# Acelogic/LTX-2-MLX

Measured on AMD Instinct MI355X. Metric: denoise_steps_per_sec, higher is better.
Workload: dtype bf16; 1 GPU; LTX-2 19B distilled DiT (48 layers, D=4096, 32x128 heads), 768x512x65 (N=3456 video tokens, S=1024 text tokens), 8-step distilled sigmas, bf16, random-init weights; parallelism=prompt-parallel x1 (independent prompt/seed per GPU, one RCCL weight broadcast)

## Files before the change

### ltx-2-mlx_amd/csrc/gemm_v4.hip

```cpp
#include <stdlib.h>

#include "gemm_epilogue.h"
#include "gemm_v4_loop.inc"

namespace {

typedef unsigned int u32x8 __attribute__((ext_vector_type(8)));
typedef unsigned int u32x16 __attribute__((ext_vector_type(16)));

#define V4_INS_DENSE : "{v[0:15]}"(voffA), "{v[16:23]}"(voffB), "{v[24:27]}"(addrA), "{v[28:31]}"(addrB), [ra] "s"(ra), [rw] "s"(rw), \
                       [nk] "s"(nk), [la] "s"(la), [lw] "s"(lw), [kb] "s"(kb)
#define V4_INS_CONV V4_INS_DENSE, "{v32}"(tapv), [lcpt] "s"(lcpt), [cptm1] "s"(cptm1)
#define V4_OUT16                                                                                                          \
    "={a[0:15]}"(acc[0]), "={a[16:31]}"(acc[1]), "={a[32:47]}"(acc[2]), "={a[48:63]}"(acc[3]), "={a[64:79]}"(acc[4]),   \
        "={a[80:95]}"(acc[5]), "={a[96:111]}"(acc[6]), "={a[112:127]}"(acc[7]), "={a[128:143]}"(acc[8]),                 \
        "={a[144:159]}"(acc[9]), "={a[160:175]}"(acc[10]), "={a[176:191]}"(acc[11]), "={a[192:207]}"(acc[12]),          \
        "={a[208:223]}"(acc[13]), "={a[224:239]}"(acc[14]), "={a[240:255]}"(acc[15])
#define V4_ASM(LOOP) asm volatile(LOOP : V4_OUT16 V4_INS_DENSE : LTX2_V4_CLOBBERS)
#define V4_ASM_CONV(LOOP) asm volatile(LOOP : V4_OUT16 V4_INS_CONV : LTX2_V4_CLOBBERS)

template <int LAYOUT, int BM, bool W8 = false>
struct V4Geo {
    static constexpr bool L41 = LAYOUT == 4 || LAYOUT == 7;
    static constexpr int BN = LAYOUT == 4 ? 128 : LAYOUT == 7 ? 64 : 256;
    static_assert(LAYOUT == 3 || LAYOUT == 4 || LAYOUT == 5 || LAYOUT == 6 || LAYOUT == 7, "wave layout");
    static constexpr int MB = LAYOUT == 5 ? 32 : 16;
    static constexpr bool L14 = !L41;
    static constexpr int WM = L41 ? BM / 4 : BM;
    static constexpr int WN = LAYOUT == 4 ? 128 : 64;
    static constexpr int RBW = (WM + MB - 1) / MB, CBW = WN / MB;
    static constexpr int NKS = MB == 16 ? 2 : 4;
    static constexpr int WROW = W8 ? 64 : 128;
    static constexpr int NPA = BM / 32, NPW = BN * WROW / 4096;
    static constexpr int A_STAGE = L41 ? BM * 128 : 32768, W_BASE = 2 * A_STAGE, W_STAGE = BN * WROW;
    static_assert(!W8 || LAYOUT == 3, "fp8-resident weights run on layout 3");
    static constexpr int LOOP_BYTES = W_BASE + 2 * W_STAGE;
    static constexpr int EPI_BYTES = 4 * WM * WN * 2;
    static constexpr int LDS_BYTES = LOOP_BYTES > EPI_BYTES ? LOOP_BYTES : EPI_BYTES;
    static_assert(LAYOUT == 4 ? (BM == 384 || BM == 448 || BM == 512) : LAYOUT == 7 ? BM == 512 : (BM == 224 || BM == 256), "tile rows");
    static_assert(LAYOUT != 6 || BM == 224, "layout 6 tile rows");
    static_assert(LDS_BYTES <= 160 * 1024, "LDS");
};

template <int EPI, int LAYOUT, int BM, bool CONV, int VAR>
__device__ __forceinline__ void gemm_v4_tile(const GemmParams& p, const int bid) {
    constexpr bool W8 = VAR == 20;
    constexpr bool F8 = LAYOUT == 5 || LAYOUT == 6;
    using G = V4Geo<LAYOUT, BM, W8>;
    constexpr int TBN = G::BN, NPA = G::NPA, NPW = G::NPW, MB = G::MB, WM = G::WM, WN = G::WN, RBW = G::RBW, CBW = G::CBW, NKS = G::NKS;
    static_assert(!CONV || !(LAYOUT == 5 || LAYOUT == 6), "conv runs on the bf16 layouts");
    extern __shared__ __attribute__((aligned(16))) char smem[];
    const unsigned lds0 = (unsigned)(uintptr_t)(lds_ptr_t)smem;
    const int tid = threadIdx.x;
    const int lane = tid & 63;
    const int w = __builtin_amdgcn_readfirstlane(tid >> 6);
    const int wr = G::L41 ? w : 0, wc = G::L41 ? 0 : w;
#ifdef LTX2_V4_PROBE
    const unsigned long long t_k0 = __builtin_amdgcn_s_memtime();
#endif

    constexpr bool FOLD_OK = LAYOUT == 3 && !CONV && VAR == 30;
    constexpr bool FOLD_CONS = FOLD_OK && (EPI == EPI_BF16 || EPI == EPI_GELU_BF16);
    constexpr bool FOLD_PROD = FOLD_OK && EPI == EPI_RESID_GATE_F32;
    const int Mt = (p.M + BM - 1) / BM, Nt = LAYOUT == 7 ? 1 : p.N / TBN;
    const int ntiles = Mt * Nt;
    const int split = p.splitk > 1 ? bid / ntiles : 0;
    const int id = xcd_remap(bid - split * ntiles, ntiles);
    constexpr int GROUP = 8;
    const int per_group = GROUP * Nt;
    const int g = id / per_group;
    const int first_m = g * GROUP;
    const int gsz = min(Mt - first_m, GROUP);
    const int rem = id - g * per_group;
    const int m0 = (first_m + rem % gsz) * BM;
    const int n0 = (rem / gsz) * TBN;

    u32x16 voffA = {0, 0, 0, 0, 0, 0, 0, 0, 0, 0, 0, 0, 0, 0, 0, 0};
    u32x8 voffB = {0, 0, 0, 0, 0, 0, 0, 0};
    const int Hp = p.H + 2, Wp = p.Wd + 2;
    constexpr bool SHORT_OK = LAYOUT == 3 && BM == 224 && !CONV;
    const int valid_rows = p.M - m0;
    const int short_rb = !SHORT_OK ? 0 : valid_rows <= 96 ? 6 : valid_rows <= 160 ? 10 : 0;
    const int npa_rt = short_rb ? short_rb / 2 : NPA;
#pragma unroll
    for (int j = 0; j < NPA; ++j) {
        const int r = (w * npa_rt + j) * 8 + (lane >> 3);
        const int chunk = (lane & 7) ^ ((r >> 1) & 7);
        const int m = min(m0 + r, p.M - 1);
        if constexpr (CONV) {
            const int hw = p.H * p.Wd;
            const int t = m / hw, r2 = m - t * hw, h = r2 / p.Wd, x = r2 - h * p.Wd;
            voffA[j] = (unsigned)((t * Hp + h) * Wp + x) * (unsigned)(p.Cin * 2) + chunk * 16;
        } else {
            voffA[j] = (unsigned)m * (unsigned)(p.lda * (F8 ? 1 : 2)) + chunk * 16;
        }
    }
#pragma unroll
    for (int j = 0; j < NPW; ++j) {
        if constexpr (W8) {
            const int r = (w * NPW + j) * 16 + (lane >> 2);
            const int c8 = (2 * (lane & 3)) ^ (2 * ((r >> 2) & 3));
            voffB[j] = (unsigned)(n0 + r) * (unsigned)p.K + c8 * 8;
        } else {
            const int r = (w * NPW + j) * 8 + (lane >> 3);
            const int chunk = (lane & 7) ^ ((r >> 1) & 7);
            const int wrow = LAYOUT == 7 ? min(n0 + r, p.N - 1) : n0 + r;
            voffB[j] = (unsigned)wrow * (unsigned)(p.K * (F8 ? 1 : 2)) + chunk * 16;
        }
    }
    const int lr = lane & (MB - 1), kq = lane / MB;
    const int xbase = kq ^ ((lr >> 1) & 7);
    u32x4 addrA = {0, 0, 0, 0}, addrB = {0, 0, 0, 0};
    if constexpr (F8) {
#pragma unroll
        for (int q = 0; q < 4; ++q) {
            const unsigned c = (unsigned)((4 * (q >> 1) + 2 * kq + (q & 1)) ^ ((lr >> 1) & 7)) << 4;
            addrA[q] = lds0 + (wr * WM + lr) * 128 + c;
            addrB[q] = lds0 + G::W_BASE + (wc * WN + lr) * 128 + c;
        }
    }
#pragma unroll
    for (int ks = 0; ks < (F8 ? 0 : NKS); ++ks) {
        const unsigned c = (unsigned)(((MB == 32 ? 2 : 4) * ks) ^ xbase) << 4;
        const unsigned a0 = lds0 + (wr * WM + lr) * 128 + c;
        const unsigned b0 = W8 ? lds0 + G::W_BASE + (wc * WN + lr) * 64 + ((unsigned)((4 * ks + kq) ^ (2 * ((lr >> 2) & 3))) << 3)
                               : lds0 + G::W_BASE + (wc * WN + lr) * 128 + c;
        if constexpr (MB == 16) {
            addrA[ks] = a0;
            addrA[ks + 2] = a0 + G::A_STAGE;
            addrB[ks] = b0;
            addrB[ks + 2] = b0 + G::W_STAGE;
        } else {
            addrA[ks] = a0;
            addrB[ks] = b0;
        }
    }
    const __amdgpu_buffer_rsrc_t ra = __builtin_amdgcn_make_buffer_rsrc(F8 ? (void*)p.A8 : (void*)p.A, 0, 0x7fffffff, 0x00020000);
    const __amdgpu_buffer_rsrc_t rw = __builtin_amdgcn_make_buffer_rsrc((W8 || F8) ? (void*)p.W8 : (void*)p.W, 0, 0x7fffffff, 0x00020000);
    const unsigned la = __builtin_amdgcn_readfirstlane(lds0 + w * npa_rt * 1024);
    const unsigned lw = __builtin_amdgcn_readfirstlane(lds0 + G::W_BASE + w * NPW * 1024);
    const unsigned nkt = p.K / (F8 ? 128 : 64);
    const unsigned kb = __builtin_amdgcn_readfirstlane(p.splitk > 1 ? 2 * ((unsigned)split * (nkt / 2) / (unsigned)p.splitk) : 0u);
    const unsigned nk = __builtin_amdgcn_readfirstlane(p.splitk > 1 ? 2 * (((unsigned)split + 1) * (nkt / 2) / (unsigned)p.splitk) - kb : nkt);
    unsigned tapv = 0;
    unsigned lcpt = 0, cptm1 = 0;
    if constexpr (CONV) {
        const int ntap = 9 * p.taps_t;
        const int a = p.taps_t == 3 ? lane / 9 : 0, bc = p.taps_t == 3 ? lane % 9 : lane;
        tapv = lane < ntap ? (unsigned)((a * Hp + bc / 3) * Wp + bc % 3) * (unsigned)(p.Cin * 2) : 0u;
        lcpt = __builtin_amdgcn_readfirstlane(p.cin_shift - 6);
        cptm1 = __builtin_amdgcn_readfirstlane((p.Cin >> 6) - 1);
    }

    constexpr int NG = MB == 32 ? 4 : 1;
    constexpr bool HOIST_COL_VECTORS = LAYOUT == 3 && MB == 16 && BM == 224 && !CONV &&
                                       (EPI == EPI_BF16 || EPI == EPI_GELU_BF16 || EPI == EPI_RESID_GATE_F32);
    f32x4 bias4[CBW][NG];
    f32x4 gate4[CBW][NG];
    auto load_bias = [&]() __attribute__((always_inline)) {
#pragma unroll
        for (int cb = 0; cb < CBW; ++cb)
#pragma unroll
            for (int gq = 0; gq < NG; ++gq)
                bias4[cb][gq] = (p.bias && (LAYOUT != 7 || n0 + wc * WN + cb * MB + 8 * gq + 4 * kq < p.N)) ? *(const f32x4*)(p.bias + n0 + wc * WN + cb * MB + 8 * gq + 4 * kq)
                                                                                                                  : f32x4{0.f, 0.f, 0.f, 0.f};
    };
    auto load_gate = [&]() __attribute__((always_inline)) {
#pragma unroll
        for (int cb = 0; cb < CBW; ++cb)
#pragma unroll
            for (int gq = 0; gq < NG; ++gq)
                gate4[cb][gq] = (EPI == EPI_RESID_GATE_F32 && p.gate_table) ? *(const f32x4*)(p.gate_table + n0 + wc * WN + cb * MB + 8 * gq + 4 * kq)
                                                                             : f32x4{0.f, 0.f, 0.f, 0.f};
    };
    constexpr int RF_OFF = G::LOOP_BYTES, RF_FAC = RF_OFF + GEMM_RF_MAX_PARTS * BM * 4;
    if constexpr (FOLD_CONS) {
        if (p.rf_parts) {
            const __amdgpu_buffer_rsrc_t rp = __builtin_amdgcn_make_buffer_rsrc((void*)p.rf_parts, 0, 0x7fffffff, 0x00020000);
            const int total = p.rf_nparts * (BM / 4);
            for (int it = 0; it * 256 < total; ++it) {
                const int idx = it * 256 + tid;
                if (idx < total) {
                    const int part = idx / (BM / 4), c4 = idx - part * (BM / 4);
                    const unsigned voff = (unsigned)(((long)part * p.rf_ld + m0 + 4 * c4) * 4);
#if defined(__HIP_DEVICE_COMPILE__)
                    __builtin_amdgcn_raw_ptr_buffer_load_lds(rp, (lds_ptr_t)(smem + RF_OFF + it * 4096 + w * 1024), 16, voff, 0, 0, 0);
#else
                    (void)voff;
#endif
                }
            }
        }
    }
    [[maybe_unused]] float rf[FOLD_CONS ? RBW : 1];
    if constexpr (HOIST_COL_VECTORS) load_bias();
    constexpr bool RESID_LDS_OK = EPI == EPI_RESID_GATE_F32 && (LAYOUT == 3 || LAYOUT == 5 || LAYOUT == 6) && VAR != 9;
    constexpr bool RESID_PRELOAD = RESID_LDS_OK && LAYOUT == 3 && BM == 224 && !W8 && !CONV;
    constexpr int ROWB = WN * 4, PR = 32, RPP = PR / MB, NP = RBW / RPP, NIT = PR / 4;
    const bool rowgate = p.gate && p.gate_stride != 0;
    const int rr = lane >> 4, cc = lane & 15;
    float* xg = (float*)p.out + (long)(m0 + rr) * p.ldo + n0 + wc * WN + cc * 4;
    const int nparts = min(NP, (p.M - m0 + PR - 1) / PR);
    const float* gg = rowgate ? p.gate + (long)(m0 + rr) * p.gate_stride + n0 + wc * WN + cc * 4 : nullptr;
    constexpr int X0_OFF = G::LOOP_BYTES;
    if constexpr (RESID_PRELOAD) {
        if (!rowgate) {
            const __amdgpu_buffer_rsrc_t rx = __builtin_amdgcn_make_buffer_rsrc((void*)p.out, 0, 0x7fffffff, 0x00020000);
#pragma unroll
            for (int i = 0; i < NIT; ++i) {
                const long grow = min((long)m0 + i * 4 + rr, (long)p.M - 1);
                const unsigned voff = (unsigned)((grow * p.ldo + n0 + wc * WN + cc * 4) * 4);
#if defined(__HIP_DEVICE_COMPILE__)
                __builtin_amdgcn_raw_ptr_buffer_load_lds(rx, (lds_ptr_t)(smem + X0_OFF + w * (PR * ROWB) + i * 1024), 16, voff, 0, 0, 0);
#else
                (void)voff;
#endif
            }
        }
    }
    f32x16 acc[16];
#ifdef LTX2_V4_PROBE
    const unsigned long long t_loop0 = __builtin_amdgcn_s_memtime();
#endif
    if constexpr (W8) {
        u32x8 scl;
#pragma unroll
        for (int cb = 0; cb < 4; ++cb) {
            const float sv = p.wscale[n0 + wc * WN + cb * MB + lr];
            scl[2 * cb] = scl[2 * cb + 1] = __builtin_bit_cast(unsigned, sv);
        }
        if constexpr (BM == 224) {
            if (short_rb == 6)
                asm volatile(LTX2_V4_L14_M16_RB6_W8 : V4_OUT16 V4_INS_DENSE, LTX2_V4_L14_M16_RB6_W8_SCL(scl) : LTX2_V4_L14_M16_RB6_W8_CLOBBERS);
            else if (short_rb == 10)
                asm volatile(LTX2_V4_L14_M16_RB10_W8 : V4_OUT16 V4_INS_DENSE, LTX2_V4_L14_M16_RB10_W8_SCL(scl) : LTX2_V4_L14_M16_RB10_W8_CLOBBERS);
            else
                asm volatile(LTX2_V4_L14_M16_RB14_W8 : V4_OUT16 V4_INS_DENSE, LTX2_V4_L14_M16_RB14_W8_SCL(scl) : LTX2_V4_L14_M16_RB14_W8_CLOBBERS);
        } else
            asm volatile(LTX2_V4_L14_M16_RB16_W8 : V4_OUT16 V4_INS_DENSE, LTX2_V4_L14_M16_RB16_W8_SCL(scl) : LTX2_V4_L14_M16_RB16_W8_CLOBBERS);
    } else if constexpr (CONV) {
        if constexpr (LAYOUT == 3) {
            if constexpr (BM == 224) V4_ASM_CONV(LTX2_V4_L14_M16_RB14_CONV);
            else V4_ASM_CONV(LTX2_V4_L14_M16_RB16_CONV);
        } else {
            if constexpr (LAYOUT == 7) V4_ASM_CONV(LTX2_V4_L41N_M16_RB8_CONV);
            else if constexpr (BM == 384) V4_ASM_CONV(LTX2_V4_L41_M16_RB6_CONV);
            else if constexpr (BM == 448) V4_ASM_CONV(LTX2_V4_L41_M16_RB7_CONV);
            else V4_ASM_CONV(LTX2_V4_L41_M16_RB8_CONV);
        }
    } else if constexpr (LAYOUT == 3) {
        if constexpr (BM == 224) {
            if (short_rb == 6) V4_ASM(LTX2_V4_L14_M16_RB6);
            else if (short_rb == 10) V4_ASM(LTX2_V4_L14_M16_RB10);
            else V4_ASM(LTX2_V4_L14_M16_RB14);
        } else {
#ifdef LTX2_V4_PROBE
            if constexpr (VAR == 1) V4_ASM(LTX2_V4_L14_M16_RB16_NODMA);
            else if constexpr (VAR == 2) V4_ASM(LTX2_V4_L14_M16_RB16_NOREAD);
            else
#endif
                V4_ASM(LTX2_V4_L14_M16_RB16);
        }
    } else if constexpr (LAYOUT == 4) {
        if constexpr (BM == 448) V4_ASM(LTX2_V4_L41_M16_RB7);
        else V4_ASM(LTX2_V4_L41_M16_RB8);
    } else if constexpr (LAYOUT == 6) {
        static_assert(BM == 224, "layout 6 tile rows");
        V4_ASM(LTX2_V4_F8_M16_RB14);
    } else {
        if constexpr (BM == 224) V4_ASM(LTX2_V4_F8_RB7);
        else V4_ASM(LTX2_V4_F8_RB8);
    }
#ifdef LTX2_V4_PROBE
    const unsigned long long t_loop1 = __builtin_amdgcn_s_memtime();
    if (p.dbg && bid == 0 && tid == 0) {
        ((unsigned long long*)p.dbg)[0] = t_loop1 - t_loop0;
        ((unsigned long long*)p.dbg)[2] = t_loop0 - t_k0;
    }
#endif

    GemmParams pe = p;
    if (EPI == EPI_F32 && p.splitk > 1) pe.out = (float*)p.out + (long)split * p.M * p.ldo;
    if constexpr (!HOIST_COL_VECTORS) load_bias();
    [[maybe_unused]] int lr_e = lr, tid_e = tid;
    if constexpr (FOLD_OK) asm volatile("" : "+v"(lr_e), "+v"(tid_e));
    if constexpr (FOLD_CONS) {
        if (p.rf_parts && tid_e < BM) {
            const float* pl = (const float*)(smem + RF_OFF);
            float sq = 0.f;
            for (int j = 0; j < p.rf_nparts; ++j) sq += pl[j * BM + tid_e];
            *(float*)(smem + RF_FAC + tid_e * 4) = rsqrtf(sq / (float)p.rf_dim + p.rf_eps);
        }
    }
    load_gate();
#pragma unroll
    for (int cb = 0; cb < CBW; ++cb)
#pragma unroll
        for (int gq = 0; gq < NG; ++gq) {
            asm volatile("" : "+v"(bias4[cb][gq]));
            if (EPI == EPI_RESID_GATE_F32) asm volatile("" : "+v"(gate4[cb][gq]));
        }
    float as_row[F8 ? RBW : 1];
    f32x4 ws4[F8 ? CBW : 1][NG];
    if constexpr (F8) {
#pragma unroll
        for (int rb = 0; rb < RBW; ++rb) as_row[rb] = p.ascale[min(m0 + wr * WM + rb * MB + lr, p.M - 1)];
#pragma unroll
        for (int cb = 0; cb < CBW; ++cb)
#pragma unroll
            for (int gq = 0; gq < NG; ++gq) ws4[cb][gq] = *(const f32x4*)(p.wscale + n0 + wc * WN + cb * MB + 8 * gq + 4 * kq);
    }
    auto acc_group = [&](int rb, int cb, int gq) -> f32x4 {
        const int blk = rb * CBW + cb;
        if constexpr (F8 && MB == 32) {
            const f32x16& a = acc[blk];
            return f32x4{a[4 * gq], a[4 * gq + 1], a[4 * gq + 2], a[4 * gq + 3]} * (ws4[cb][gq] * as_row[rb]);
        } else if constexpr (F8) {
            const f32x16& a = acc[blk >> 2];
            const int o = (blk & 3) * 4;
            return f32x4{a[o], a[o + 1], a[o + 2], a[o + 3]} * (ws4[cb][gq] * as_row[rb]);
        } else if constexpr (MB == 32) {
            const f32x16& a = acc[blk];
            return f32x4{a[4 * gq], a[4 * gq + 1], a[4 * gq + 2], a[4 * gq + 3]};
        } else {
            const f32x16& a = acc[blk >> 2];
            const int o = (blk & 3) * 4;
            return f32x4{a[o], a[o + 1], a[o + 2], a[o + 3]};
        }
    };
    constexpr bool BF16_OUT = EPI == EPI_BF16 || EPI == EPI_GELU_BF16 || EPI == EPI_SILU_BF16;
    const bool resid_lds = RESID_LDS_OK;
    if constexpr (RESID_LDS_OK) {
      if (resid_lds) {
        static_assert(RBW % RPP == 0 && ROWB == 256 && 4 * 2 * PR * ROWB <= G::LDS_BYTES, "resid epilogue slab");
        auto run = [&](auto RG) __attribute__((always_inline)) {
            constexpr bool ROWGATE = decltype(RG)::value;
            f32x4 g4[CBW][NG];
#pragma unroll
            for (int cb = 0; cb < CBW; ++cb)
#pragma unroll
                for (int gq = 0; gq < NG; ++gq) {
                    g4[cb][gq] = f32x4{1.f, 1.f, 1.f, 1.f};
                    if (!ROWGATE && (p.gate || p.gate_table)) {
                        g4[cb][gq] = gate4[cb][gq];
                        if (p.gate) g4[cb][gq] += *(const f32x4*)(p.gate + n0 + wc * WN + cb * MB + 8 * gq + 4 * kq);
                    }
                }
            char* wl = smem + w * (2 * PR * ROWB);
            f32x4 gtab = {0.f, 0.f, 0.f, 0.f};
            if (ROWGATE && p.gate_table) gtab = *(const f32x4*)(p.gate_table + n0 + wc * WN + cc * 4);
            const bool shadow = FOLD_PROD && !ROWGATE && p.shadow != nullptr;
            f32x4 sm4 = {1.f, 1.f, 1.f, 1.f};
            bf16* yg = nullptr;
            float* sspart = (float*)(smem + 4 * (2 * PR * ROWB)) + w * BM;
            if constexpr (FOLD_PROD && !ROWGATE) {
                if (shadow) {
                    if (p.shadow_scale) sm4 += *(const f32x4*)(p.shadow_scale + n0 + wc * WN + cc * 4);
                    yg = p.shadow + (long)(m0 + rr) * p.ld_shadow + n0 + wc * WN + cc * 4;
                }
            }
            f32x4 xv[3][NIT];
            [[maybe_unused]] f32x4 gv[ROWGATE ? 3 : 1][NIT];
            auto load_part = [&](auto PART) __attribute__((always_inline)) {
                constexpr int part = decltype(PART)::value, slot = part % 3;
#pragma unroll
                for (int i = 0; i < NIT; ++i) {
                    const long grow = min((long)m0 + part * PR + i * 4 + rr, (long)p.M - 1) - (m0 + rr);
                    xv[slot][i] = *(const f32x4*)(xg + grow * p.ldo);
                    if constexpr (ROWGATE) gv[slot][i] = *(const f32x4*)(gg + grow * p.gate_stride);
                }
            };
            if constexpr (RESID_PRELOAD && !ROWGATE) {
#pragma unroll
                for (int i = 0; i < NIT; ++i) xv[0][i] = *(const f32x4*)(smem + X0_OFF + w * (PR * ROWB) + i * 1024 + lane * 16);
            } else {
                load_part(std::integral_constant<int, 0>{});
            }
            if (nparts > 1) load_part(std::integral_constant<int, 1>{});
            __syncthreads();
            static_for<0, NP>([&](auto PART) __attribute__((always_inline)) {
                constexpr int part = decltype(PART)::value;
                if (part < nparts) {
                    char* sl = wl + (part & 1) * (PR * ROWB);
#pragma unroll
                    for (int r = 0; r < RPP; ++r) {
                        const int rb = part * RPP + r, row = r * MB + lr;
#pragma unroll
                        for (int cb = 0; cb < CBW; ++cb)
#pragma unroll
                            for (int gq = 0; gq < NG; ++gq) {
                                const f32x4 v = g4[cb][gq] * (acc_group(rb, cb, gq) + bias4[cb][gq]);
                                const int chunk = (cb * MB + 8 * gq + 4 * kq) >> 2;
                                *(f32x4*)(sl + row * ROWB + ((chunk ^ (row & 15)) << 4)) = v;
                            }
                    }
                    if constexpr (part + 2 < NP) {
                        if (part + 2 < nparts) load_part(std::integral_constant<int, part + 2>{});
                    }
#pragma unroll
                    for (int i = 0; i < NIT; ++i) {
                        const int row = i * 4 + rr;
                        asm volatile("" : "+v"(xv[part % 3][i]));
                        f32x4 d = *(const f32x4*)(sl + row * ROWB + ((cc ^ (row & 15)) << 4));
                        if constexpr (ROWGATE) d *= gtab + gv[part % 3][i];
                        const f32x4 xn = xv[part % 3][i] + d;
                        const bool live = m0 + part * PR + row < p.M;
                        if (live) *(f32x4*)(xg + ((long)part * PR + row - rr) * p.ldo) = xn;
                        if constexpr (FOLD_PROD && !ROWGATE) {
                            if (shadow) {
                                float ss = (xn[0] * xn[0] + xn[1] * xn[1]) + (xn[2] * xn[2] + xn[3] * xn[3]);
                                ss += dpp_f32<0xB1>(ss);
                                ss += dpp_f32<0x4E>(ss);
                                ss += dpp_f32<0x141>(ss);
                                ss += dpp_f32<0x140>(ss);
                                const f32x4 y = xn * sm4;
                                if (live) {
                                    *(bf16x4*)(yg + ((long)part * PR + row - rr) * p.ld_shadow) = pack_bf16x4(y[0], y[1], y[2], y[3]);
                                }
                                if (cc == 0) sspart[part * PR + row] = ss;
                            }
                        }
                    }
                }
            });
            if constexpr (FOLD_PROD && !ROWGATE) {
                if (shadow) {
                    __syncthreads();
                    const float* sp = (const float*)(smem + 4 * (2 * PR * ROWB));
                    if (tid < BM && m0 + tid < p.M) p.shadow_ss[(long)(n0 / TBN) * p.ld_ss + m0 + tid] = (sp[tid] + sp[BM + tid]) + (sp[2 * BM + tid] + sp[3 * BM + tid]);
                }
            }
        };
        if (rowgate) run(std::true_type{});
        else run(std::false_type{});
      }
    }
    if constexpr (EPI == EPI_RESID_GATE_F32) {
      if (!resid_lds) {
        constexpr int RBH = (RBW + 1) / 2;
#pragma unroll
        for (int half = 0; half < 2; ++half) {
            f32x4 xs[RBH][CBW][NG];
#pragma unroll
            for (int r = 0; r < RBH; ++r) {
                const int rb = half * RBH + r;
                if (rb >= RBW || wr * WM + rb * MB >= BM || m0 + wr * WM + rb * MB >= p.M) continue;
                const int row = min(m0 + wr * WM + rb * MB + lr, p.M - 1);
#pragma unroll
                for (int cb = 0; cb < CBW; ++cb)
#pragma unroll
                    for (int gq = 0; gq < NG; ++gq)
                        xs[r][cb][gq] = *(const f32x4*)((const float*)p.out + (long)row * p.ldo + (n0 + wc * WN + cb * MB + 8 * gq + 4 * kq));
            }
#pragma unroll
            for (int r = 0; r < RBH; ++r) {
                const int rb = half * RBH + r;
                if (rb >= RBW || wr * WM + rb * MB >= BM || m0 + wr * WM + rb * MB >= p.M) continue;
                const int row = m0 + wr * WM + rb * MB + lr;
                const bool ok = row < p.M;
#pragma unroll
                for (int cb = 0; cb < CBW; ++cb)
#pragma unroll
                    for (int gq = 0; gq < NG; ++gq) {
                        asm volatile("" : "+v"(xs[r][cb][gq]));
                        const int col = n0 + wc * WN + cb * MB + 8 * gq + 4 * kq;
                        const f32x4 v = acc_group(rb, cb, gq) + bias4[cb][gq];
                        f32x4 gt = {1.f, 1.f, 1.f, 1.f};
                        if (p.gate || p.gate_table) {
                            gt = gate4[cb][gq];
                            if (p.gate && ok) gt += *(const f32x4*)(p.gate + (long)row * p.gate_stride + col);
                        }
                        if (ok) *(f32x4*)((float*)p.out + (long)row * p.ldo + col) = xs[r][cb][gq] + gt * v;
                    }
            }
        }
      }
    } else if constexpr (VAR != 9 && (BF16_OUT || EPI == EPI_ADD_BF16)) {
        constexpr int ROWB = WN * 2, CPR = ROWB / 16, RPI = 64 / CPR;
        __syncthreads();
        if constexpr (FOLD_CONS) {
#pragma unroll
            for (int rb = 0; rb < RBW; ++rb) rf[rb] = p.rf_parts ? *(const float*)(smem + RF_FAC + (rb * MB + lr_e) * 4) : 1.f;
        }
        char* wl = smem + w * (WM * ROWB);
        if constexpr (EPI == EPI_ADD_BF16) {
            const __amdgpu_buffer_rsrc_t rr = __builtin_amdgcn_make_buffer_rsrc((void*)p.res, 0, 0x7fffffff, 0x00020000);
#pragma unroll
            for (int it = 0; it < WM / RPI; ++it) {
                const int r = it * RPI + lane / CPR, c = lane % CPR;
                const int sw = CPR == 8 ? ((r >> 1) & 7) : (r & 15);
                const int row = min(m0 + wr * WM + r, p.M - 1);
                const unsigned voff = (unsigned)(((long)row * p.ldres + n0 + wc * WN + (c ^ sw) * 8) * 2);
#if defined(__HIP_DEVICE_COMPILE__)
                __builtin_amdgcn_raw_ptr_buffer_load_lds(rr, (lds_ptr_t)(wl + it * 1024), 16, voff, 0, 0, 0);
#else
                (void)voff;
#endif
            }
            asm volatile("s_waitcnt vmcnt(0)" ::: "memory");
        }
#pragma unroll
        for (int rb = 0; rb < RBW; ++rb) {
            if (m0 + wr * WM + rb * MB >= p.M) continue;
            const int r = rb * MB + lr;
            const int sw = CPR == 8 ? ((r >> 1) & 7) : (r & 15);
            [[maybe_unused]] bf16x4 rsv[CBW][NG];
            if constexpr (EPI == EPI_ADD_BF16) {
#pragma unroll
                for (int cb = 0; cb < CBW; ++cb)
#pragma unroll
                    for (int gq = 0; gq < NG; ++gq) {
                        const int byte = (cb * MB + 8 * gq + 4 * kq) * 2;
                        rsv[cb][gq] = *(const bf16x4*)(wl + r * ROWB + (((byte >> 4) ^ sw) << 4) + (byte & 15));
                    }
            }
#pragma unroll
            for (int cb = 0; cb < CBW; ++cb)
#pragma unroll
              for (int gq = 0; gq < NG; ++gq) {
                f32x4 v;
                if constexpr (FOLD_CONS) {
                    v = acc_group(rb, cb, gq) * rf[rb] + bias4[cb][gq];
                } else {
                    v = acc_group(rb, cb, gq) + bias4[cb][gq];
                }
                if (EPI == EPI_GELU_BF16) {
                    const f32x2 g0 = gelu_tanh2(f32x2{v[0], v[1]}), g1 = gelu_tanh2(f32x2{v[2], v[3]});
                    v = f32x4{g0[0], g0[1], g1[0], g1[1]};
                }
                if (EPI == EPI_SILU_BF16) v = f32x4{silu_f(v[0]), silu_f(v[1]), silu_f(v[2]), silu_f(v[3])};
                const int byte = (cb * MB + 8 * gq + 4 * kq) * 2;
                const int chunk = (byte >> 4) ^ sw;
                bf16x4* slot = (bf16x4*)(wl + r * ROWB + chunk * 16 + (byte & 15));
                if constexpr (EPI == EPI_ADD_BF16) {
                    const bf16x4 rs = rsv[cb][gq];
                    v += f32x4{bf2f(rs[0]), bf2f(rs[1]), bf2f(rs[2]), bf2f(rs[3])};
                }
                *slot = pack_bf16x4(v[0], v[1], v[2], v[3]);
              }
        }
        if ((LAYOUT == 3 || LAYOUT == 5 || LAYOUT == 6) && EPI == EPI_BF16 && !CONV && p.vt && n0 >= p.vt_col0) {
            const int cw = n0 + wc * WN - p.vt_col0;
            const int head = cw / p.vt_hd, d0 = cw - head * p.vt_hd;
            bf16* vrow = p.vt + (long)head * p.vt_head_stride + (long)(d0 + (lane >> 2)) * p.vt_npad + m0;
#pragma unroll 1
            for (int dg = 0; dg < WN / 16; ++dg) {
                const int c = dg * 16 + (lane >> 2);
                const int coff = (c & 7) * 2, cchunk = c >> 3;
#pragma unroll
                for (int cg = 0; cg < BM / 32; ++cg) {
                    const int ch = cg * 4 + (lane & 3);
                    const int kbase = (ch >> 2) * 32 + (ch & 3) * 4;
                    constexpr int RUN2 = 16;
                    bf16x8 v;
#pragma unroll
                    for (int e = 0; e < 8; ++e) {
                        const int r = kbase + (e >> 2) * RUN2 + (e & 3);
                        const bf16 x = *(const bf16*)(wl + r * ROWB + ((cchunk ^ ((r >> 1) & 7)) << 4) + coff);
                        v[e] = (m0 + r < p.M) ? x : f2bf(0.f);
                    }
                    if (m0 + ch * 8 < p.vt_npad) *(bf16x8*)(vrow + (long)dg * 16 * p.vt_npad + ch * 8) = v;
                }
            }
        } else {
            constexpr int RBATCH = 4;
            static_assert((WM / RPI) % RBATCH == 0, "readback batches");
            u32x4 rbv[RBATCH];
#pragma unroll
            for (int it = 0; it < WM / RPI; ++it) {
                const int r = it * RPI + lane / CPR, c = lane % CPR;
                if (it % RBATCH == 0) {
#pragma unroll
                    for (int b = 0; b < RBATCH; ++b) {
                        const int rb2 = (it + b) * RPI + lane / CPR;
                        const int sw2 = CPR == 8 ? ((rb2 >> 1) & 7) : (rb2 & 15);
                        rbv[b] = *(const u32x4*)(wl + rb2 * ROWB + ((c ^ sw2) << 4));
                    }
                }
                const u32x4 v = rbv[it % RBATCH];
                const int row = m0 + wr * WM + r;
                if (row < p.M && (LAYOUT != 7 || n0 + wc * WN + c * 8 < p.N)) *(u32x4*)((bf16*)p.out + (long)row * p.ldo + n0 + wc * WN + c * 8) = v;
                if constexpr (EPI == EPI_BF16 && !CONV && (LAYOUT == 3 || LAYOUT == 5 || LAYOUT == 6)) {
                    if (p.rowss) {
                        const bf16x8 h = as_bf16x8(v);
                        float ss = 0.f;
#pragma unroll
                        for (int e = 0; e < 8; ++e) ss += bf2f(h[e]) * bf2f(h[e]);
                        ss += __shfl_xor(ss, 1);
                        ss += __shfl_xor(ss, 2);
                        ss += __shfl_xor(ss, 4);
                        if (c == 0 && row < p.M) p.rowss[(long)row * (p.N / 64) + (n0 + wc * WN) / 64] = ss;
                    }
                }
            }
        }
    } else if constexpr (EPI == EPI_D2S_BF16 && CONV && LAYOUT == 3) {
        const int colw = n0 + wc * WN;
        const int s_idx = colw >> p.cf_shift, c_base = colw & (p.Cf - 1);
        const int fhw = p.fh * p.fw;
        const int da = s_idx / fhw, db = (s_idx - da * fhw) / p.fw, dd = s_idx - da * fhw - db * p.fw;
        const int sp = p.ft * fhw, cmask = p.c_d2s - 1;
        const bf16* xs = p.res ? p.res : p.A;
        const int Ho = p.H * p.fh, Wo = p.Wd * p.fw;
        int row = m0 + lr;
        const int hw = p.H * p.Wd;
        int pt = row / hw, ph = (row - pt * hw) / p.Wd, pw = row - pt * hw - ph * p.Wd;
#pragma unroll
        for (int rb = 0; rb < RBW; ++rb, row += MB) {
            if (rb) {
                pw += MB;
                while (pw >= p.Wd) {
                    pw -= p.Wd;
                    if (++ph >= p.H) {
                        ph = 0;
                        ++pt;
                    }
                }
            }
            const int to = pt * p.ft + da - p.drop_first;
            const bool ok = row < p.M && to >= 0;
            unsigned short rs[CBW][4];
            if (p.d2s_residual) {
                const bf16* xr = xs + (long)min(row, p.M - 1) * p.Cin + s_idx;
#pragma unroll
                for (int cb = 0; cb < CBW; ++cb)
#pragma unroll
                    for (int e = 0; e < 4; ++e) rs[cb][e] = *(const unsigned short*)(xr + ((c_base + cb * MB + 4 * kq + e) & cmask) * sp);
            }
            bf16* orow = (bf16*)p.out + (((long)to * Ho + (ph * p.fh + db)) * Wo + (pw * p.fw + dd)) * p.Cf + c_base + 4 * kq;
#pragma unroll
            for (int cb = 0; cb < CBW; ++cb) {
                f32x4 v = acc_group(rb, cb, 0) + bias4[cb][0];
                if (p.d2s_residual) {
#pragma unroll
                    for (int e = 0; e < 4; ++e) v[e] += bf2f(__builtin_bit_cast(bf16, rs[cb][e]));
                }
                if (ok) *(bf16x4*)(orow + cb * MB) = pack_bf16x4(v[0], v[1], v[2], v[3]);
            }
        }
    } else {
#pragma unroll
        for (int rb = 0; rb < RBW; ++rb) {
            if (wr * WM + rb * MB >= BM) continue;
            const int row = m0 + wr * WM + rb * MB + lr;
            if (row >= p.M) continue;
            const EpiRow er = epi_row_setup<EPI>(p, row);
#pragma unroll
            for (int cb = 0; cb < CBW; ++cb)
#pragma unroll
                for (int gq = 0; gq < NG; ++gq) {
                    const int col = n0 + wc * WN + cb * MB + 8 * gq + 4 * kq;
                    epi_store4<EPI>(pe, er, row, col, acc_group(rb, cb, gq), bias4[cb][gq], gate4[cb][gq]);
                }
        }
    }
#ifdef LTX2_V4_PROBE
    if (p.dbg && bid == 0 && tid == 0) ((unsigned long long*)p.dbg)[1] = __builtin_amdgcn_s_memtime() - t_k0;
#endif
}

template <int EPI, int LAYOUT, int BM, bool CONV, int VAR>
__global__ __launch_bounds__(256) void gemm_v4_kernel(const GemmParams p) {
    gemm_v4_tile<EPI, LAYOUT, BM, CONV, VAR>(p, (int)blockIdx.x);
}

template <int EPI, int LAYOUT, int BM, bool CONV = false, int VAR = 0>
int launch_v4(const GemmParams& p, hipStream_t stream) {
    using G = V4Geo<LAYOUT, BM, VAR == 20>;
    constexpr int LDS = G::LDS_BYTES + ((EPI == EPI_RESID_GATE_F32 && LAYOUT == 3 && BM == 224 && !CONV && VAR != 20 && VAR != 9) ? 32768 : 0) +
                        ((LAYOUT == 3 && !CONV && VAR == 30 && (EPI == EPI_BF16 || EPI == EPI_GELU_BF16)) ? (GEMM_RF_MAX_PARTS + 1) * BM * 4 : 0);
    static_assert(LDS <= 160 * 1024, "LDS");
    static PerDeviceOnce attr_once;
    if (attr_once.first()) {
        (void)hipFuncSetAttribute((const void*)gemm_v4_kernel<EPI, LAYOUT, BM, CONV, VAR>, hipFuncAttributeMaxDynamicSharedMemorySize, LDS);
    }
    const int Mt = (p.M + BM - 1) / BM, Nt = LAYOUT == 7 ? 1 : p.N / G::BN;
    hipLaunchKernelGGL((gemm_v4_kernel<EPI, LAYOUT, BM, CONV, VAR>), dim3(Mt * Nt * (p.splitk > 1 ? p.splitk : 1)), dim3(256), LDS, stream, p);
    LTX2_CHECK_LAUNCH("gemm_v4_kernel");
    return LTX2_OK;
}

__global__ __launch_bounds__(256) void splitk_reduce_kernel(const float* __restrict__ part, int splits, long mn, int N, const float* __restrict__ bias,
                                                            const bf16* __restrict__ res, bf16* __restrict__ out) {
    for (long i = ((long)blockIdx.x * blockDim.x + threadIdx.x) * 4; i < mn; i += (long)gridDim.x * blockDim.x * 4) {
        f32x4 a = *(const f32x4*)(part + i);
        for (int s = 1; s < splits; ++s) a += *(const f32x4*)(part + (long)s * mn + i);
        const int n = (int)(i % N);
        if (bias) a += *(const f32x4*)(bias + n);
        if (res) {
            const bf16x4 r = *(const bf16x4*)(res + i);
            a += f32x4{bf2f(r[0]), bf2f(r[1]), bf2f(r[2]), bf2f(r[3])};
        }
        *(bf16x4*)(out + i) = pack_bf16x4(a[0], a[1], a[2], a[3]);
    }
}

constexpr unsigned epi_bit(int e) { return 1u << e; }
constexpr unsigned EPIS_DENSE = epi_bit(EPI_BF16) | epi_bit(EPI_GELU_BF16) | epi_bit(EPI_SILU_BF16) | epi_bit(EPI_F32) | epi_bit(EPI_RESID_GATE_F32) | epi_bit(EPI_ADD_BF16);
constexpr unsigned EPIS_FP8 = epi_bit(EPI_BF16) | epi_bit(EPI_GELU_BF16) | epi_bit(EPI_F32) | epi_bit(EPI_RESID_GATE_F32);
constexpr unsigned EPIS_FOLD = epi_bit(EPI_BF16) | epi_bit(EPI_GELU_BF16) | epi_bit(EPI_RESID_GATE_F32);
constexpr unsigned EPIS_L4 = epi_bit(EPI_BF16) | epi_bit(EPI_ADD_BF16);

template <int LAYOUT, int BM, int VAR, unsigned EPIS>
int launch_v4_dense(const GemmParams& p, int epilogue, hipStream_t stream) {
    return gemm_epilogue_dispatch(epilogue, [&](auto E) {
        constexpr int e = decltype(E)::value;
        if constexpr ((EPIS >> e) & 1) return launch_v4<e, LAYOUT, BM, false, VAR>(p, stream);
        else return (int)LTX2_E_INVALID;
    });
}

struct V4Dense {
    GemmV4Kernel k;
    unsigned epis;
    int (*launch)(const GemmParams&, int, hipStream_t);
};
template <int LAYOUT, int BM, int VAR, unsigned EPIS>
constexpr V4Dense v4_dense() { return {{LAYOUT, BM, VAR}, EPIS, launch_v4_dense<LAYOUT, BM, VAR, EPIS>}; }
const V4Dense V4_DENSE[] = {
    v4_dense<3, 224, 0, EPIS_DENSE>(), v4_dense<3, 256, 0, EPIS_DENSE>(), v4_dense<3, 224, 30, EPIS_FOLD>(), v4_dense<3, 256, 30, EPIS_FOLD>(),
    v4_dense<3, 224, 20, EPIS_FP8>(),  v4_dense<3, 256, 20, EPIS_FP8>(),  v4_dense<4, 448, 0, EPIS_L4>(),    v4_dense<4, 512, 0, EPIS_L4>(),
    v4_dense<5, 224, 0, EPIS_FP8>(),   v4_dense<5, 256, 0, EPIS_FP8>(),   v4_dense<6, 224, 0, EPIS_FP8>(),
};

}

bool gemm_v4_supported(const GemmParams& p, int epilogue, bool conv) {
    if (conv || epilogue == EPI_D2S_BF16) return false;
    if (p.N % 256 != 0 || p.K % 128 != 0 || p.K < 256 || p.M < 1024) return false;
    if ((long)p.M * p.lda * 2 >= (1L << 31) || (long)p.N * p.K * 2 >= (1L << 31)) return false;
    if (p.ldo % 8 != 0 || ((uintptr_t)p.out & 15)) return false;
    if (epilogue == EPI_ADD_BF16 && (!p.res || (long)p.M * p.ldres * 2 >= (1L << 31) || p.ldres % 8 != 0 || ((uintptr_t)p.res & 15))) return false;
    return true;
}

bool gemm_v4_vt_supported(const GemmParams& p, int epilogue, int bm) {
    if (epilogue != EPI_BF16 || !p.vt) return false;
    if (p.vt_col0 % 256 != 0 || (p.vt_hd != 64 && p.vt_hd != 128) || (p.N - p.vt_col0) % p.vt_hd != 0) return false;
    if (p.vt_npad % 64 != 0 || p.vt_npad < p.M) return false;
    return (long)((p.M + bm - 1) / bm) * bm >= p.vt_npad;
}

bool gemm_v4_w8_supported(const GemmParams& p, int epilogue) {
    if (epilogue != EPI_BF16 && epilogue != EPI_GELU_BF16 && epilogue != EPI_F32 && epilogue != EPI_RESID_GATE_F32) return false;
    if (p.N % 256 != 0 || p.K % 128 != 0 || p.K < 256 || p.M < 1) return false;
    if ((long)p.M * p.lda * 2 >= (1L << 31) || (long)p.N * p.K >= (1L << 31)) return false;
    if (p.ldo % 8 != 0 || ((uintptr_t)p.out & 15) || ((uintptr_t)p.W8 & 15)) return false;
    return true;
}

bool gemm_v4_f8_supported(const GemmParams& p, int epilogue) {
    if (epilogue != EPI_BF16 && epilogue != EPI_GELU_BF16 && epilogue != EPI_F32 && epilogue != EPI_RESID_GATE_F32) return false;
    if (!p.A8 || !p.ascale || !p.W8 || !p.wscale) return false;
    if (p.N % 256 != 0 || p.K % 256 != 0 || p.K < 512 || p.M < 1) return false;
    if ((long)p.M * p.lda >= (1L << 31) || (long)p.N * p.K >= (1L << 31)) return false;
    if (p.lda % 16 != 0 || p.ldo % 8 != 0 || ((uintptr_t)p.out & 15) || ((uintptr_t)p.W8 & 15) || ((uintptr_t)p.A8 & 15)) return false;
    return true;
}

int gemm_v4_launch(const GemmParams& p, int epilogue, hipStream_t stream, GemmV4Kernel k) {
    if (k.layout == 5 || k.layout == 6)
        LTX2_CHECK_ARG(gemm_v4_f8_supported(p, epilogue), "gemm_v4: fp8 compute needs A8 + ascale + W8 + wscale, N %% 256 == 0, K %% 256 == 0, K >= 512, a dense bf16/gelu/f32/residual epilogue (N=%d K=%d epilogue=%d)", p.N, p.K, epilogue);
    else if (k.var == 20)
        LTX2_CHECK_ARG(p.wscale && gemm_v4_w8_supported(p, epilogue), "gemm_v4: fp8-resident weights need N %% 256 == 0, K %% 128 == 0, K >= 256, a dense bf16/gelu/f32/residual epilogue (N=%d K=%d epilogue=%d)", p.N, p.K, epilogue);
    else if (k.layout == 4)
        LTX2_CHECK_ARG(p.N % 128 == 0, "gemm_v4 layout 4: N %% 128");
    for (const V4Dense& d : V4_DENSE) {
        if (d.k.layout != k.layout || d.k.bm != k.bm || d.k.var != k.var) continue;
        if (epilogue >= 0 && epilogue < EPI_COUNT && ((d.epis >> epilogue) & 1)) return d.launch(p, epilogue, stream);
        ltx2_set_error(k.layout == 4 ? "gemm_v4 layout 4: unsupported epilogue %d" : k.var == 30 ? "gemm_v4: a folded norm on epilogue %d" : "gemm_v4: unsupported epilogue %d", epilogue);
        return LTX2_E_INVALID;
    }
    ltx2_set_error("gemm_v4: wave layout %d (3 = bf16 dense, 4 = 128-column convs, 5 = fp8 compute)", k.layout);
    return LTX2_E_INVALID;
}

bool gemm_v4_conv_supported(const GemmParams& p, int epilogue) {
    if (epilogue != EPI_BF16 && epilogue != EPI_ADD_BF16 && epilogue != EPI_D2S_BF16) return false;
    if (epilogue == EPI_D2S_BF16 && (p.N % 256 != 0 || p.Cf < 64 || (p.Cf & (p.Cf - 1)) || (p.d2s_residual && (!p.res || p.c_d2s < 1 || (p.c_d2s & (p.c_d2s - 1)))))) return false;
#ifdef LTX2_NO_CONV7
    const bool narrow = false;
#else
    const bool narrow = epilogue == EPI_BF16 && p.N <= 64 && p.N % 8 == 0 && p.N >= 8 && p.ldo == p.N;
#endif
    if (p.Cin < 128 || (p.Cin & (p.Cin - 1)) || (p.N % 128 != 0 && !narrow)) return false;
    if (p.taps_t != 3 && p.taps_t != 1) return false;
    if (p.M < 512) return false;
    if ((long)(p.T + 2) * (p.H + 2) * (p.Wd + 2) * p.Cin * 2 >= (1L << 31) || (long)p.N * p.K * 2 >= (1L << 31)) return false;
    if (p.ldo % 8 != 0 || ((uintptr_t)p.out & 15)) return false;
    if (epilogue == EPI_ADD_BF16 && (!p.res || (long)p.M * p.ldres * 2 >= (1L << 31) || p.ldres % 8 != 0 || ((uintptr_t)p.res & 15))) return false;
    return true;
}

static int conv_splits(long tiles, int nk, long mn, long ws_bytes, double* cost_out = nullptr) {
    int best = 1;
    double best_cost = (double)((tiles + 255) / 256) * (nk + 6);
    for (int s = 2; s <= 16; ++s) {
        const int h = nk / 2, lo = 2 * (h / s), hi = 2 * ((h + s - 1) / s);
        if (lo < 8 || (long)s * mn * 4 > ws_bytes) break;
        const double cost = (double)((tiles * s + 255) / 256) * (hi + 6) + 3.0 + (double)s * (double)mn / 1.44e6;
        if (cost < best_cost * 0.97) {
            best_cost = cost;
            best = s;
        }
    }
    if (cost_out) *cost_out = best_cost;
    return best;
}

int gemm_v4_conv_launch(const GemmParams& p_in, int epilogue, hipStream_t stream, void* splitk_ws, long ws_bytes) {
    GemmParams p = p_in;
    LTX2_CHECK_ARG(gemm_v4_conv_supported(p, epilogue), "gemm_v4 conv: unsupported problem (Cin=%d N=%d M=%d epilogue=%d)", p.Cin, p.N, p.M, epilogue);
    p.splitk = 1;
    if (p.N <= 64) return launch_v4<EPI_BF16, 7, 512, true>(p, stream);
    if (p.N % 256 != 0) {
        long best_cost = 0;
        int bm = 512;
        for (const int cand : {512, 448, 384}) {
            const long tiles = ((long)p.M + cand - 1) / cand * (p.N / 128), cost = (tiles + 255) / 256 * cand;
            if (!best_cost || cost < best_cost) {
                best_cost = cost;
                bm = cand;
            }
        }
#define CONV4(E) (bm == 512 ? launch_v4<E, 4, 512, true>(p, stream) : bm == 448 ? launch_v4<E, 4, 448, true>(p, stream) : launch_v4<E, 4, 384, true>(p, stream))
        if (epilogue == EPI_BF16) return CONV4(EPI_BF16);
        return CONV4(EPI_ADD_BF16);
#undef CONV4
    }
    const long t256 = ((long)(p.M + 255) / 256) * (p.N / 256), t224 = ((long)(p.M + 223) / 224) * (p.N / 256);
    bool b224 = (t224 + 255) / 256 * 224 < (t256 + 255) / 256 * 256 || t224 < 256;
    const long mn = (long)p.M * p.N;
    if (epilogue == EPI_D2S_BF16) return b224 ? launch_v4<EPI_D2S_BF16, 3, 224, true>(p, stream) : launch_v4<EPI_D2S_BF16, 3, 256, true>(p, stream);
    int splits = 1;
    if (splitk_ws && p.ldo == p.N) {
        double c224 = 0, c256 = 0;
        const int s224 = conv_splits(t224, p.K / 64, mn, ws_bytes, &c224), s256 = conv_splits(t256, p.K / 64, mn, ws_bytes, &c256);
        if (s224 > 1 || s256 > 1) b224 = c224 * 224 <= c256 * 256;
        splits = b224 ? s224 : s256;
    }
    if (splits > 1) {
        GemmParams q = p;
        q.splitk = splits;
        q.out = splitk_ws;
        q.bias = nullptr;
        q.res = nullptr;
        const int rc = b224 ? launch_v4<EPI_F32, 3, 224, true>(q, stream) : launch_v4<EPI_F32, 3, 256, true>(q, stream);
        if (rc != LTX2_OK) return rc;
        const long want = (mn / 4 + 255) / 256;
        hipLaunchKernelGGL(splitk_reduce_kernel, dim3((unsigned)(want < 4096 ? want : 4096)), dim3(256), 0, stream, (const float*)splitk_ws, splits, mn,
                           p.N, p.bias, epilogue == EPI_ADD_BF16 ? p.res : nullptr, (bf16*)p.out);
        LTX2_CHECK_LAUNCH("splitk_reduce_kernel");
        return LTX2_OK;
    }
    if (epilogue == EPI_BF16) return b224 ? launch_v4<EPI_BF16, 3, 224, true>(p, stream) : launch_v4<EPI_BF16, 3, 256, true>(p, stream);
    return b224 ? launch_v4<EPI_ADD_BF16, 3, 224, true>(p, stream) : launch_v4<EPI_ADD_BF16, 3, 256, true>(p, stream);
}

#ifdef LTX2_V4_PROBE
int gemm_v4_probe_launch(const GemmParams& p, GemmV4Kernel k, hipStream_t stream) {
    if (k.layout == 3 && k.bm == 224 && k.var == 9) return launch_v4<EPI_BF16, 3, 224, false, 9>(p, stream);
    if (k.layout == 3 && k.bm == 256 && k.var == 1) return launch_v4<EPI_BF16, 3, 256, false, 1>(p, stream);
    if (k.layout == 3 && k.bm == 256 && k.var == 2) return launch_v4<EPI_BF16, 3, 256, false, 2>(p, stream);
    ltx2_set_error("gemm_v4 probe: no ablation kernel of layout %d, %d rows, variant %d", k.layout, k.bm, k.var);
    return LTX2_E_INVALID;
}
#endif
```

Before: 13.50 steps/s.

## Burst-prefetch residual parts into LDS via buffer DMA in gated-residual epilogue

In the residual-gate epilogue, the next two residual parts are fetched straight into the now-free W-stage LDS buffers with buffer_load_lds before the barrier. This replaces per-part register prefetch and deepens the prefetch pipeline, with hand-placed vmcnt waits. The row-sum partials move into the X0 region, and the broadcast gate vector is loaded early alongside the gate table so its global load comes off the epilogue path. The risks are higher LDS pressure and the fragility of hand-tuned wait counts, which are tied to NIT==8.

Measured after the change: 13.53 steps/s, median of 6. About the same (+0.2%).

```diff
diff --git a/ltx-2-mlx_amd/csrc/gemm_v4.hip b/ltx-2-mlx_amd/csrc/gemm_v4.hip
--- a/ltx-2-mlx_amd/csrc/gemm_v4.hip
+++ b/ltx-2-mlx_amd/csrc/gemm_v4.hip
@@ -2,6 +2,10 @@
 
 #include "gemm_epilogue.h"
 #include "gemm_v4_loop.inc"
+
+#ifndef LTX2_RESID_BURST
+#define LTX2_RESID_BURST 1
+#endif
 
 namespace {
 
@@ -157,6 +161,8 @@
                                        (EPI == EPI_BF16 || EPI == EPI_GELU_BF16 || EPI == EPI_RESID_GATE_F32);
     f32x4 bias4[CBW][NG];
     f32x4 gate4[CBW][NG];
+    constexpr bool BCAST_GATE_HOISTED = EPI == EPI_RESID_GATE_F32 && LAYOUT == 3 && BM == 224 && !CONV && VAR != 20 && VAR != 9 && LTX2_RESID_BURST;
+    [[maybe_unused]] f32x4 gateb4[BCAST_GATE_HOISTED ? CBW : 1][NG];
     auto load_bias = [&]() __attribute__((always_inline)) {
 #pragma unroll
         for (int cb = 0; cb < CBW; ++cb)
@@ -172,6 +178,13 @@
             for (int gq = 0; gq < NG; ++gq)
                 gate4[cb][gq] = (EPI == EPI_RESID_GATE_F32 && p.gate_table) ? *(const f32x4*)(p.gate_table + n0 + wc * WN + cb * MB + 8 * gq + 4 * kq)
                                                                              : f32x4{0.f, 0.f, 0.f, 0.f};
+        if constexpr (BCAST_GATE_HOISTED) {
+#pragma unroll
+            for (int cb = 0; cb < CBW; ++cb)
+#pragma unroll
+                for (int gq = 0; gq < NG; ++gq)
+                    gateb4[cb][gq] = (p.gate && p.gate_stride == 0) ? *(const f32x4*)(p.gate + n0 + wc * WN + cb * MB + 8 * gq + 4 * kq) : f32x4{0.f, 0.f, 0.f, 0.f};
+        }
     };
     constexpr int RF_OFF = G::LOOP_BYTES, RF_FAC = RF_OFF + GEMM_RF_MAX_PARTS * BM * 4;
     if constexpr (FOLD_CONS) {
@@ -254,7 +267,7 @@
             else if (short_rb == 10) V4_ASM(LTX2_V4_L14_M16_RB10);
             else V4_ASM(LTX2_V4_L14_M16_RB14);
         } else {
-#ifdef LTX2_V4_PROBE
+#if defined(LTX2_V4_PROBE) && defined(LTX2_V4_L14_M16_RB16_NODMA)
             if constexpr (VAR == 1) V4_ASM(LTX2_V4_L14_M16_RB16_NODMA);
             else if constexpr (VAR == 2) V4_ASM(LTX2_V4_L14_M16_RB16_NOREAD);
             else
@@ -299,6 +312,7 @@
         for (int gq = 0; gq < NG; ++gq) {
             asm volatile("" : "+v"(bias4[cb][gq]));
             if (EPI == EPI_RESID_GATE_F32) asm volatile("" : "+v"(gate4[cb][gq]));
+            if constexpr (BCAST_GATE_HOISTED) asm volatile("" : "+v"(gateb4[cb][gq]));
         }
     float as_row[F8 ? RBW : 1];
     f32x4 ws4[F8 ? CBW : 1][NG];
@@ -343,7 +357,11 @@
                     g4[cb][gq] = f32x4{1.f, 1.f, 1.f, 1.f};
                     if (!ROWGATE && (p.gate || p.gate_table)) {
                         g4[cb][gq] = gate4[cb][gq];
-                        if (p.gate) g4[cb][gq] += *(const f32x4*)(p.gate + n0 + wc * WN + cb * MB + 8 * gq + 4 * kq);
+                        if constexpr (BCAST_GATE_HOISTED) {
+                            if (p.gate) g4[cb][gq] += gateb4[cb][gq];
+                        } else {
+                            if (p.gate) g4[cb][gq] += *(const f32x4*)(p.gate + n0 + wc * WN + cb * MB + 8 * gq + 4 * kq);
+                        }
                     }
                 }
             char* wl = smem + w * (2 * PR * ROWB);
@@ -352,7 +370,12 @@
             const bool shadow = FOLD_PROD && !ROWGATE && p.shadow != nullptr;
             f32x4 sm4 = {1.f, 1.f, 1.f, 1.f};
             bf16* yg = nullptr;
-            float* sspart = (float*)(smem + 4 * (2 * PR * ROWB)) + w * BM;
+            constexpr bool BURST = RESID_PRELOAD && !ROWGATE && LTX2_RESID_BURST;
+            constexpr int XW_OFF = G::W_BASE, XW_STRIDE = G::W_STAGE, NDMA = 2;
+            static_assert(!BURST || (G::W_STAGE == 4 * PR * ROWB && NDMA == 2), "burst: a wave's share of a W stage holds one part");
+            constexpr int SS_STRIDE = BURST ? PR * ROWB / 4 : BM;
+            float* const ssbase = (float*)(smem + (BURST ? X0_OFF : 4 * (2 * PR * ROWB)));
+            float* sspart = ssbase + w * SS_STRIDE;
             if constexpr (FOLD_PROD && !ROWGATE) {
                 if (shadow) {
                     if (p.shadow_scale) sm4 += *(const f32x4*)(p.shadow_scale + n0 + wc * WN + cc * 4);
@@ -370,14 +393,35 @@
                     if constexpr (ROWGATE) gv[slot][i] = *(const f32x4*)(gg + grow * p.gate_stride);
                 }
             };
-            if constexpr (RESID_PRELOAD && !ROWGATE) {
-#pragma unroll
-                for (int i = 0; i < NIT; ++i) xv[0][i] = *(const f32x4*)(smem + X0_OFF + w * (PR * ROWB) + i * 1024 + lane * 16);
+            if constexpr (BURST) {
+                const __amdgpu_buffer_rsrc_t rx = __builtin_amdgcn_make_buffer_rsrc((void*)p.out, 0, 0x7fffffff, 0x00020000);
+                static_for<1, 1 + NDMA>([&](auto PART) __attribute__((always_inline)) {
+                    constexpr int part = decltype(PART)::value;
+                    if (part < nparts) {
+#pragma unroll
+                        for (int i = 0; i < NIT; ++i) {
+                            const long grow = min((long)m0 + part * PR + i * 4 + rr, (long)p.M - 1);
+                            const unsigned voff = (unsigned)((grow * p.ldo + n0 + wc * WN + cc * 4) * 4);
+#if defined(__HIP_DEVICE_COMPILE__)
+                            __builtin_amdgcn_raw_ptr_buffer_load_lds(rx, (lds_ptr_t)(smem + XW_OFF + (part - 1) * XW_STRIDE + w * (PR * ROWB) + i * 1024), 16, voff, 0, 0, 0);
+#else
+                            (void)voff;
+#endif
+                        }
+                    }
+                });
+                asm volatile("" ::: "memory");
             } else {
-                load_part(std::integral_constant<int, 0>{});
-            }
-            if (nparts > 1) load_part(std::integral_constant<int, 1>{});
-            __syncthreads();
+                if constexpr (RESID_PRELOAD && !ROWGATE) {
+#pragma unroll
+                    for (int i = 0; i < NIT; ++i) xv[0][i] = *(const f32x4*)(smem + X0_OFF + w * (PR * ROWB) + i * 1024 + lane * 16);
+                } else {
+                    load_part(std::integral_constant<int, 0>{});
+                }
+                if (nparts > 1) load_part(std::integral_constant<int, 1>{});
+            }
+            if constexpr (BURST) asm volatile("s_waitcnt lgkmcnt(0)\n\ts_barrier" ::: "memory");
+            else __syncthreads();
             static_for<0, NP>([&](auto PART) __attribute__((always_inline)) {
                 constexpr int part = decltype(PART)::value;
                 if (part < nparts) {
@@ -394,16 +438,32 @@
                                 *(f32x4*)(sl + row * ROWB + ((chunk ^ (row & 15)) << 4)) = v;
                             }
                     }
-                    if constexpr (part + 2 < NP) {
-                        if (part + 2 < nparts) load_part(std::integral_constant<int, part + 2>{});
+                    if constexpr (!BURST) {
+                        if constexpr (part + 2 < NP) {
+                            if (part + 2 < nparts) load_part(std::integral_constant<int, part + 2>{});
+                        }
+                    } else if constexpr (part <= NDMA && part + 3 < NP) {
+                        if (part + 3 < nparts) load_part(std::integral_constant<int, part + 3>{});
+                    }
+                    if constexpr (BURST && part == 0) {
+                        static_assert(NIT == 8, "burst wait counts");
+                        if (3 < nparts) asm volatile("s_waitcnt vmcnt(8)" ::: "memory");
+                        else asm volatile("s_waitcnt vmcnt(0)" ::: "memory");
                     }
 #pragma unroll
                     for (int i = 0; i < NIT; ++i) {
                         const int row = i * 4 + rr;
-                        asm volatile("" : "+v"(xv[part % 3][i]));
+                        f32x4 xi;
+                        if constexpr (BURST && part <= NDMA) {
+                            constexpr int off = part == 0 ? X0_OFF : XW_OFF + (part - 1) * XW_STRIDE;
+                            xi = *(const f32x4*)(smem + off + w * (PR * ROWB) + i * 1024 + lane * 16);
+                        } else {
+                            asm volatile("" : "+v"(xv[part % 3][i]));
+                            xi = xv[part % 3][i];
+                        }
                         f32x4 d = *(const f32x4*)(sl + row * ROWB + ((cc ^ (row & 15)) << 4));
                         if constexpr (ROWGATE) d *= gtab + gv[part % 3][i];
-                        const f32x4 xn = xv[part % 3][i] + d;
+                        const f32x4 xn = xi + d;
                         const bool live = m0 + part * PR + row < p.M;
                         if (live) *(f32x4*)(xg + ((long)part * PR + row - rr) * p.ldo) = xn;
                         if constexpr (FOLD_PROD && !ROWGATE) {
@@ -421,13 +481,25 @@
                             }
                         }
                     }
+                    if constexpr (BURST && part > NDMA && part + 3 < NP) {
+                        if (part + 3 < nparts) load_part(std::integral_constant<int, part + 3>{});
+                    }
+#ifdef LTX2_V4_PROBE
+                    if constexpr (part == 0) {
+                        if (p.dbg && bid == 0 && tid == 0) ((unsigned long long*)p.dbg)[3] = __builtin_amdgcn_s_memtime() - t_loop1;
+                    }
+#endif
                 }
             });
+#ifdef LTX2_V4_PROBE
+            if (p.dbg && bid == 0 && tid == 0) ((unsigned long long*)p.dbg)[4] = __builtin_amdgcn_s_memtime() - t_loop1;
+#endif
             if constexpr (FOLD_PROD && !ROWGATE) {
                 if (shadow) {
                     __syncthreads();
-                    const float* sp = (const float*)(smem + 4 * (2 * PR * ROWB));
-                    if (tid < BM && m0 + tid < p.M) p.shadow_ss[(long)(n0 / TBN) * p.ld_ss + m0 + tid] = (sp[tid] + sp[BM + tid]) + (sp[2 * BM + tid] + sp[3 * BM + tid]);
+                    const float* sp = ssbase;
+                    if (tid < BM && m0 + tid < p.M)
+                        p.shadow_ss[(long)(n0 / TBN) * p.ld_ss + m0 + tid] = (sp[tid] + sp[SS_STRIDE + tid]) + (sp[2 * SS_STRIDE + tid] + sp[3 * SS_STRIDE + tid]);
                 }
             }
         };
```
